# jgiovatto/srsLTE

Measured on AMD Instinct MI355X. Metric: turbo decoded Mbit/s (LTE 20 MHz, K=6144, 8 half-iterations) incl. OFDM demod of the same subframes, higher is better.
Workload: dtype int16

## Files before the change

srslte_amd/csrc/turbo_kernels.hip:

```cpp
#include <type_traits>

#include "hip_common.h"
#include "turbo_arith.h"
#include "turbo_device.h"

namespace phyhip {
namespace turbo {

typedef uint32_t u4v __attribute__((ext_vector_type(4)));
template <bool NT>
__device__ __forceinline__ uint4 ws_load16(const void* p)
{
  if constexpr (NT) {
    const u4v v = __builtin_nontemporal_load(reinterpret_cast<const u4v*>(p));
    return make_uint4(v.x, v.y, v.z, v.w);
  } else {
    return *reinterpret_cast<const uint4*>(p);
  }
}

template <class AR>
__device__ __forceinline__ void beta_step(s2 (&o)[8], s2 x, s2 y)
{
  auto adds = [](s2 a, s2 b) { return AR::add_raw(a, b); };
// ... 371 lines not shown
            y0[j] = (uint32_t)(uint16_t)AR::conv_in(r[0][3 * j + 1]) | ((uint32_t)(uint16_t)AR::conv_in(r[1][3 * j + 1]) << 16);
            y1[j] = (uint32_t)(uint16_t)AR::conv_in(r[0][3 * j + 2]) | ((uint32_t)(uint16_t)AR::conv_in(r[1][3 * j + 2]) << 16);
          }
          const uint32_t slot = (b0 + lb) * 64 + cw * LPC + pp;
          store_block_v<AR::kIs8>(S, slot, sv);
          store_block_v<AR::kIs8>(P0, slot, y0);
          store_block_v<AR::kIs8>(P1, slot, y1);
        }
      }
    }
  }
  if (pp == 0) {
    const short* in = in_wave + (size_t)(g < n_cb_left ? g : n_cb_left - 1) * in_stride;
    short*       TL = TL_wave + 16 * g;
#pragma unroll
    for (int i = 0; i < 3; i++) {
      TL[i]     = AR::conv_in(in[3 * K + 2 * i]);
      TL[3 + i] = AR::conv_in(in[3 * K + 2 * i + 1]);
      TL[6 + i] = AR::conv_in(in[3 * K + 6 + 2 * i]);
      TL[9 + i] = AR::conv_in(in[3 * K + 6 + 2 * i + 1]);
    }
  }
}

template <int LPC, class AR>
__device__ __forceinline__ void extract_input_sb16(const short* in, uint32_t K, uint32_t nblk, int lane, int pl, uint32_t* S,
                                                   uint32_t* P0, uint32_t* P1, short* TL, uint32_t* stage)
{
  constexpr int  NB  = 2 * LPC;
  const int      cbw = lane / LPC;
  uint4*         st4 = reinterpret_cast<uint4*>(stage);
  auto put = [&](uint32_t* dst, uint32_t b, const uint4& lo, const uint4& hi) {
    st4[cbw * 2 * LPC + pl]       = lo;
    st4[cbw * 2 * LPC + LPC + pl] = hi;
    uint32_t r[8];
#pragma unroll
    for (int j = 0; j < 8; j++) {
      const uint32_t w = stage[cbw * 8 * LPC + j * LPC + pl];
      r[j] = (uint32_t)(uint16_t)AR::conv_in((short)(w & 0xffffu)) | ((uint32_t)(uint16_t)AR::conv_in((short)(w >> 16)) << 16);
    }
    store_block_v<AR::kIs8>(dst, b * 64 + lane, r);
  };
  for (uint32_t b = 0; b < nblk; b++) {
    const uint4* q0 = reinterpret_cast<const uint4*>(in + (size_t)b * 8 * NB);
    const uint4* q1 = reinterpret_cast<const uint4*>(in + (size_t)(K + 32) + (size_t)b * 8 * NB);
    const uint4* q2 = reinterpret_cast<const uint4*>(in + (size_t)2 * (K + 32) + (size_t)b * 8 * NB);
    const uint4  s_lo = q0[pl], s_hi = q0[LPC + pl];
    const uint4  y_lo = q1[pl], y_hi = q1[LPC + pl];
    const uint4  z_lo = q2[pl], z_hi = q2[LPC + pl];
    put(S, b, s_lo, s_hi);
    put(P0, b, y_lo, y_hi);
    put(P1, b, z_lo, z_hi);
  }
  if (pl == 0) {
    const uint32_t tb = 3 * (K + 32);
#pragma unroll
    for (int i = 0; i < 3; i++) {
      TL[i]     = AR::conv_in(in[tb + 2 * i]);
      TL[3 + i] = AR::conv_in(in[tb + 2 * i + 1]);
      TL[6 + i] = AR::conv_in(in[tb + 6 + 2 * i]);
      TL[9 + i] = AR::conv_in(in[tb + 6 + 2 * i + 1]);
    }
  }
}

template <int LPC, class AR, bool ES, int CKS>
__device__ __forceinline__ void tdec_win_unit(const WinParams& p, const uint32_t wb, const uint32_t slab, const int lane, uint4 (&Bl)[8][2][64],
                                              uint32_t (&Tr)[512])
{
  const uint32_t crc_poly = ES ? p.crc_poly : 0u;
  const CbDesc*  desc     = ES ? p.desc : nullptr;
  constexpr int  NB  = 2 * LPC;
  constexpr int  CPW = 64 / LPC;
  constexpr bool NT  = !ES && !AR::kIs8;
  static_assert(CKS == 8 || CKS == 16, "check-points every 8 or every 16 steps");
  const int     pl   = lane % LPC;
  const int     cb_raw = (int)wb * CPW + lane / LPC;
  const bool    live = cb_raw < p.n_cb;
  const int     cb   = live ? cb_raw : p.n_cb - 1;
  const uint32_t K       = p.K;
  const uint32_t long_sb = K / NB;
  const uint32_t nblk    = (long_sb + 7) >> 3;
  const uint32_t AW      = nblk * LPC * 8;

  const uint32_t AWG = AW * CPW;
  uint32_t* ws  = p.ws + (size_t)slab * p.ws_stride * CPW;
  uint32_t* S   = ws;
  uint32_t* P0  = ws + AWG;
  uint32_t* P1  = ws + 2 * AWG;
  uint32_t* A1  = ws + 3 * AWG;
  uint32_t* D   = ws + 4 * AWG;
  uint32_t* A2  = ws + 5 * AWG;
  uint32_t* CK  = ws + 6 * AWG;
  short*    TL  = reinterpret_cast<short*>(CK + (size_t)(nblk + 1) * 64 * 8) + 16 * (lane / LPC);

  if (p.n_begin == 0) {
    const bool fast = !desc && !p.in_is8 && !p.sb_layout && (long_sb & 3u) == 0 && ((reinterpret_cast<uintptr_t>(p.input) | (2u * p.in_stride)) & 7u) == 0;
    if (fast) {
      const int first = (int)wb * CPW;
      extract_input_natural16<LPC, AR>(p.input + (size_t)first * p.in_stride, p.in_stride, p.n_cb - first, K, long_sb, nblk, lane,
                                       S, P0, P1, TL - 16 * (lane / LPC), reinterpret_cast<uint2*>(&Bl[0][0][0]));
    } else if (!p.in_is8 && p.sb_layout &&
               __all(((reinterpret_cast<uintptr_t>(p.input) + 2 * (desc ? (size_t)desc[cb].in_off : (size_t)cb * p.in_stride)) & 15u) == 0)) {
      const short* in = p.input + (desc ? (size_t)desc[cb].in_off : (size_t)cb * p.in_stride);
      extract_input_sb16<LPC, AR>(in, K, long_sb >> 3, lane, pl, S, P0, P1, TL, Tr);
      if (long_sb & 7u) {
        extract_input<LPC, AR>(in, 1, K, long_sb, nblk, lane, pl, S, P0, P1, TL, long_sb >> 3, false);
      }
    } else if (p.in_is8) {
      const signed char* in = reinterpret_cast<const signed char*>(p.input) + (desc ? (size_t)desc[cb].in_off : (size_t)cb * p.in_stride);
      extract_input<LPC, AR>(in, p.sb_layout, K, long_sb, nblk, lane, pl, S, P0, P1, TL);
    } else {
      const short* in = p.input + (desc ? (size_t)desc[cb].in_off : (size_t)cb * p.in_stride);
      extract_input<LPC, AR>(in, p.sb_layout, K, long_sb, nblk, lane, pl, S, P0, P1, TL);
    }
  }
  const uint32_t wrap_row = (AR::kIs8 && (K & 31u)) ? long_sb - 1 : 0xffffffffu;
  __syncthreads();

  uint8_t*       out       = p.output + (desc ? (size_t)desc[cb].out_off : (size_t)cb * p.out_stride);
  const uint32_t out_bytes = desc ? desc[cb].out_bytes : K / 8;
  uint32_t m_own_v = ~0u, m_row_v = ~0u;
  auto     set_masks = [&](bool dead) {
    const unsigned long long dm = __ballot(dead);
    const int                og = AR::kIs8 ? ((8 * (lane & 7)) / LPC) * LPC : ((4 * (lane & 15)) / LPC) * LPC;
    m_own_v                     = dead ? 0u : ~0u;
    m_row_v                     = ((dm >> og) & 1ull) ? 0u : ~0u;
  };
  if (ES) {
    set_masks(!live);
  }
#define M_OWN (ES ? m_own_v : ~0u)
#define M_ROW (ES ? m_row_v : ~0u)
  const bool bit_rows = !ES && p.final_run && !p.dec_llr && p.n_end > p.n_begin;
  auto decide = [&](bool write, bool final_try) -> uint32_t {
    short*         o16   = (p.dec_llr && live && write) ? p.dec_llr + (size_t)cb * K : nullptr;
    const bool     whole = (long_sb & 7) == 0;
    const uint32_t bps   = long_sb >> 3;
    const uint32_t poly  = crc_poly & 0xffffffu;
    uint32_t       c0 = 0, c1 = 0;
    const uint32_t sbs  = nblk + 1;
    uint8_t*       sbuf = reinterpret_cast<uint8_t*>(&Bl[0][0][0]) + (size_t)(lane / LPC) * NB * sbs;
    static_assert(sizeof(Bl) >= 64 / LPC * 2 * LPC * (6144 / (2 * LPC) / 8 + 2), "byte image does not fit");
    if (!whole) {
      sbuf[(2 * pl) * sbs + nblk]     = 0;
      sbuf[(2 * pl + 1) * sbs + nblk] = 0;
    }
    uint4* img = &Bl[0][0][0] + (whole ? 0u : (CPW * NB * sbs + 15u) / 16u);
    if (bit_rows) {
      for (uint32_t k = lane; k < long_sb; k += 64) {
        img[k] = ws_load16<NT>(D + (size_t)k * 4);
      }
      __syncthreads();
    }
    {
      const bool wide = whole && ((bps & 3) == 0) && ((reinterpret_cast<uintptr_t>(out) & 3) == 0) && out_bytes == K / 8;
      uint32_t   w0 = 0, w1 = 0;
      uint32_t   t[8], tn[8];
      if (!bit_rows) {
        issue_rows_raw<AR::kIs8, NT>(D, 0, lane, t);
      }
      for (uint32_t b = 0; b < nblk; b++) {
        if (!bit_rows && b + 1 < nblk) {
          issue_rows_raw<AR::kIs8, NT>(D, (b + 1) & M_ROW, lane, tn);
        }
        uint32_t r[8];
        if (bit_rows) {
#pragma unroll
          for (int j = 0; j < 8; j++) {
            const uint32_t k = b * 8 + j < long_sb ? b * 8 + j : long_sb - 1;
            const uint4    m = img[k];
            r[j] = (uint32_t)(((((uint64_t)m.y << 32) | m.x) >> lane) & 1u) | ((uint32_t)(((((uint64_t)m.w << 32) | m.z) >> lane) & 1u) << 16);
          }
        } else {
          rows_to_lane_v<AR::kIs8>(Tr, lane, t, r);
        }
        uint32_t b0 = 0, b1 = 0;
#pragma unroll
        for (int j = 0; j < 8; j++) {
          if (b * 8 + j < long_sb) {
            const s2       v  = from_u(r[j]);
            const uint32_t x0 = v.x > 0 ? 1u : 0u, x1 = v.y > 0 ? 1u : 0u;
            b0 |= (x0 << 7) >> j;
            b1 |= (x1 << 7) >> j;
            if (crc_poly) {
              c0 = ((c0 << 1) & 0xffffffu) ^ ((((c0 >> 23) ^ x0) & 1u) ? poly : 0u);
              c1 = ((c1 << 1) & 0xffffffu) ^ ((((c1 >> 23) ^ x1) & 1u) ? poly : 0u);
            }
            if (o16 && whole) {
              o16[(2 * pl) * long_sb + b * 8 + j]     = AR::out16(v.x);
              o16[(2 * pl + 1) * long_sb + b * 8 + j] = AR::out16(v.y);
            }
          }
        }
        if (!whole) {
          sbuf[(2 * pl) * sbs + b]     = (uint8_t)b0;
          sbuf[(2 * pl + 1) * sbs + b] = (uint8_t)b1;
        }
        if (whole && write && live) {
          if (wide) {
            w0 |= b0 << (8 * (b & 3));
            w1 |= b1 << (8 * (b & 3));
            if ((b & 3) == 3) {
              *reinterpret_cast<uint32_t*>(out + (2 * pl) * bps + (b & ~3u))     = w0;
              *reinterpret_cast<uint32_t*>(out + (2 * pl + 1) * bps + (b & ~3u)) = w1;
              w0 = w1 = 0;
            }
          } else {
            if ((2 * pl) * bps + b < out_bytes) {
              out[(2 * pl) * bps + b] = (uint8_t)b0;
            }
            if ((2 * pl + 1) * bps + b < out_bytes) {
              out[(2 * pl + 1) * bps + b] = (uint8_t)b1;
            }
          }
        }
        if (!bit_rows) {
#pragma unroll
          for (int j = 0; j < 8; j++) {
            t[j] = tn[j];
          }
        }
      }
    }
    uint32_t crc = 0;
    if (crc_poly) {
      auto mulmod = [&](uint32_t a, uint32_t m) {
        uint32_t r = 0;
#pragma unroll 4
        for (int i = 23; i >= 0; i--) {
          r = ((r << 1) & 0xffffffu) ^ (((r >> 23) & 1u) ? poly : 0u);
          r ^= ((m >> i) & 1u) ? a : 0u;
        }
        return r;
      };
      crc = mulmod(c0, p.crc_mult[2 * pl]) ^ mulmod(c1, p.crc_mult[2 * pl + 1]);
#pragma unroll
      for (int off = LPC / 2; off > 0; off >>= 1) {
        crc ^= __shfl_xor(crc, off, LPC);
      }
    }
    __syncthreads();
    if (!whole && write && (!crc_poly || crc == 0 || final_try)) {
      const uint32_t nbytes = K / 8;
      const uint32_t lim    = out_bytes < nbytes ? out_bytes : nbytes;
      const bool     al     = (reinterpret_cast<uintptr_t>(out) & 3) == 0;
      for (uint32_t w = pl; w * 4 < nbytes; w += LPC) {
        uint32_t d = (w * 32) / long_sb, k = w * 32 - d * long_sb;
        uint32_t word = 0;
#pragma unroll
        for (int t = 0; t < 4; t++) {
          if (w * 4 + t < nbytes) {
            const uint8_t* q = sbuf + d * sbs + (k >> 3);
            uint32_t       v = ((((uint32_t)q[0] << 8) | q[1]) >> (8 - (k & 7))) & 0xffu;
            if (k + 8 > long_sb && d + 1 < (uint32_t)NB) {
              v |= (uint32_t)sbuf[(d + 1) * sbs] >> (long_sb - k);
            }
            word |= v << (8 * t);
          }
          k += 8;
          if (k >= long_sb) {
            k -= long_sb;
            d++;
          }
        }
        if (live) {
          if (al && w * 4 + 3 < lim) {
            *reinterpret_cast<uint32_t*>(out + 4 * w) = word;
          } else {
#pragma unroll
            for (int t = 0; t < 4; t++) {
              if (w * 4 + t < lim) {
                out[w * 4 + t] = (uint8_t)(word >> (8 * t));
              }
            }
          }
        }
      }
      if (o16) {
        const short* sd = reinterpret_cast<const short*>(D);
        for (uint32_t nn = pl; nn < K; nn += LPC) {
          const uint32_t d = nn / long_sb, k = nn % long_sb;
          const uint32_t e = (k * 64 + (lane / LPC) * LPC + (d >> 1)) * 2 + (d & 1);
          o16[nn] = AR::kIs8 ? (short)reinterpret_cast<const signed char*>(D)[e] : sd[e];
        }
      }
    }
    __syncthreads();
    return crc;
  };
  bool     done = false;
  uint32_t noi  = 0;

  for (uint32_t n = p.n_begin; n < p.n_end; n++) {
    const bool      dec1    = !(n & 1);
    const bool      has_app = dec1 && n > 0;
    const uint32_t* Y       = dec1 ? P0 : P1;
    const short*    xt      = dec1 ? TL : TL + 6;
    const short*    yt      = dec1 ? TL + 3 : TL + 9;

    struct Ops {
      uint32_t x[8], y[8], a[8];
    };
    auto issue = [&](uint32_t b, Ops& q) {
      if (dec1) {
        load_block_raw<AR::kIs8, NT>(S, (b & M_OWN) * 64 + lane, q.x);
      } else {
        issue_rows_raw<AR::kIs8, NT>(A2, b & M_ROW, lane, q.x);
      }
      load_block_raw<AR::kIs8, NT>(Y, (b & M_OWN) * 64 + lane, q.y);
      if (has_app) {
        issue_rows_raw<AR::kIs8, NT>(A1, b & M_ROW, lane, q.a);
      }
    };
    auto prep = [&](const Ops& q, s2(&xs)[8], s2(&ys)[8], s2(&ap)[8]) {
      uint32_t xr[8], ar[8], yr[8];
      if (dec1) {
        block_values<AR::kIs8>(q.x, xr);
      } else {
        rows_to_lane_v<AR::kIs8>(Tr, lane, q.x, xr);
      }
      if (has_app) {
        rows_to_lane_v<AR::kIs8>(Tr, lane, q.a, ar);
      }
      block_values<AR::kIs8>(q.y, yr);
#pragma unroll
      for (int j = 0; j < 8; j++) {
        xs[j] = from_u(xr[j]);
        ys[j] = from_u(yr[j]);
        ap[j] = splat(0);
        if (has_app) {
          ap[j] = from_u(ar[j]);
          xs[j] = AR::add(ap[j], xs[j]);
        }
      }
    };
    auto taken = [&](const Ops& q) {
      asm volatile("" ::"v"(q.x[0]), "v"(q.x[1]), "v"(q.x[2]), "v"(q.x[3]), "v"(q.x[4]), "v"(q.x[5]), "v"(q.x[6]), "v"(q.x[7]));
      asm volatile("" ::"v"(q.y[0]), "v"(q.y[1]), "v"(q.y[2]), "v"(q.y[3]), "v"(q.y[4]), "v"(q.y[5]), "v"(q.y[6]), "v"(q.y[7]));
      if (has_app) {
        asm volatile("" ::"v"(q.a[0]), "v"(q.a[1]), "v"(q.a[2]), "v"(q.a[3]), "v"(q.a[4]), "v"(q.a[5]), "v"(q.a[6]), "v"(q.a[7]));
      }
    };
    Ops cur, nxt, nx2;

    s2 fw[8];
#pragma unroll
    for (int i = 0; i < 8; i++) {
      fw[i] = splat(-AR::kInf);
    }
    {
      const uint32_t w0 = long_sb - TD_WIN_OVERLAP;
      const uint32_t bl = nblk - 1;
      issue(w0 >> 3, cur);
      for (uint32_t b = w0 >> 3; b <= bl; b++) {
        issue(b < bl ? b + 1 : TD_WIN_OVERLAP / 8 - 1, nxt);
        s2 xs[8], ys[8], ap[8];
        prep(cur, xs, ys, ap);
        if (b + 4 > bl) {
          const uint32_t s = b + 3 - bl;
          Bl[2 * s][0][lane]     = make_uint4(to_u(xs[0]), to_u(xs[1]), to_u(xs[2]), to_u(xs[3]));
          Bl[2 * s][1][lane]     = make_uint4(to_u(xs[4]), to_u(xs[5]), to_u(xs[6]), to_u(xs[7]));
          Bl[2 * s + 1][0][lane] = make_uint4(to_u(ys[0]), to_u(ys[1]), to_u(ys[2]), to_u(ys[3]));
          Bl[2 * s + 1][1][lane] = make_uint4(to_u(ys[4]), to_u(ys[5]), to_u(ys[6]), to_u(ys[7]));
        }
#pragma unroll
        for (int j = 0; j < 8; j++) {
          uint32_t k = b * 8 + j;
          if (k >= w0 && k < long_sb) {
            alpha_step<AR, false>(fw, fw, xs[j], ys[j]);
            uint32_t kk = k - w0;
            if (AR::norm_at(kk)) {
              AR::normalize(fw);
            }
          }
        }
        cur = nxt;
      }
    }
#pragma unroll
    for (int i = 0; i < 8; i++) {
      uint32_t u   = to_u(fw[i]);
      uint32_t prv = __shfl_up(u, 1, LPC);
      uint32_t lo  = (pl == 0) ? (uint32_t)(uint16_t)(short)(i ? -AR::kInf : 0) : (prv >> 16);
      uint32_t hi  = u & 0xffffu;
      fw[i]        = from_u(lo | (hi << 16));
    }

    s2 o[8];
#pragma unroll
    for (int i = 0; i < 8; i++) {
      o[i] = splat(-AR::kInf);
    }
    for (int b = TD_WIN_OVERLAP / 8 - 1; b >= 0; b--) {
      if (b > 0) {
        issue(b - 1, nxt);
      }
      s2 xs[8], ys[8], ap[8];
      prep(cur, xs, ys, ap);
#pragma unroll
      for (int j = 7; j >= 0; j--) {
        beta_step<AR>(o, xs[j], ys[j]);
        uint32_t k = b * 8 + j;
        if (AR::norm_at(k)) {
          AR::normalize(o);
        }
      }
      cur = nxt;
    }
    {
      short tr[8];
      tail_trellis<AR>(xt, yt, tr);
#pragma unroll
      for (int i = 0; i < 8; i++) {
        uint32_t u   = to_u(o[i]);
        uint32_t nxt = __shfl_down(u, 1, LPC);
        uint32_t lo  = u >> 16;
        uint32_t hi  = (pl == LPC - 1) ? (uint32_t)(uint16_t)tr[i] : (nxt & 0xffffu);
        o[i]         = from_u(lo | (hi << 16));
      }
      uint32_t ck[8];
#pragma unroll
      for (int i = 0; i < 8; i++) {
        ck[i] = to_u(o[i]);
      }
      store_block_v<AR::kIs8>(CK, (nblk & M_OWN) * 64 + lane, ck);
    }
    for (int b = (int)nblk - 1; b >= 0; b--) {
      const bool ahead = b + 3 <= (int)nblk;
      if (b > 1 && ahead) {
        issue(b - 2, nx2);
      }
      s2 xs[8], ys[8], ap[8];
      if (b + 4 >= (int)nblk) {
        const uint32_t s  = (uint32_t)b + 4 - nblk;
        const uint4    x0 = Bl[2 * s][0][lane], x1 = Bl[2 * s][1][lane], y0 = Bl[2 * s + 1][0][lane], y1 = Bl[2 * s + 1][1][lane];
        xs[0] = from_u(x0.x), xs[1] = from_u(x0.y), xs[2] = from_u(x0.z), xs[3] = from_u(x0.w);
        xs[4] = from_u(x1.x), xs[5] = from_u(x1.y), xs[6] = from_u(x1.z), xs[7] = from_u(x1.w);
        ys[0] = from_u(y0.x), ys[1] = from_u(y0.y), ys[2] = from_u(y0.z), ys[3] = from_u(y0.w);
        ys[4] = from_u(y1.x), ys[5] = from_u(y1.y), ys[6] = from_u(y1.z), ys[7] = from_u(y1.w);
      } else {
        prep(cur, xs, ys, ap);
      }
#pragma unroll
      for (int j = 7; j >= 0; j--) {
        uint32_t k = b * 8 + j;
        if (k < long_sb) {
          beta_step<AR>(o, xs[j], ys[j]);
          if (j == 0 && b > 0 && (CKS == 8 || !(b & 1))) {
            uint32_t ck[8];
#pragma unroll
            for (int i = 0; i < 8; i++) {
              ck[i] = to_u(o[i]);
            }
            store_block_v<AR::kIs8>(CK, ((uint32_t)b & M_OWN) * 64 + lane, ck);
          }
          if (AR::norm_at(k)) {
            AR::normalize(o);
          }
        }
      }
      if (b > 0 && ahead) {
        cur = nxt;
        nxt = nx2;
      }
    }
    __syncthreads();

#pragma unroll
    for (int i = 0; i < 8; i++) {
      o[i] = fw[i];
    }

    const uint32_t* lut = dec1 ? p.deint : p.inter;
    uint32_t*       dst = dec1 ? A2 : A1;
    const bool fuse = dec1 && n >= 2;
    const bool last = (n + 1 == p.n_end) || crc_poly;
    const bool fin  = bit_rows && n + 1 == p.n_end;

    auto rederive = [&](uint32_t b, int len, const s2(&xs)[8], const s2(&ys)[8], const uint32_t(&ckv)[8]) {
      s2 st[8];
#pragma unroll
      for (int i = 0; i < 8; i++) {
        st[i] = from_u(ckv[i]);
      }
      Bl[len - 1][0][lane] = make_uint4(ckv[0], ckv[1], ckv[2], ckv[3]);
      Bl[len - 1][1][lane] = make_uint4(ckv[4], ckv[5], ckv[6], ckv[7]);
#pragma unroll
      for (int j = 6; j >= 0; j--) {
        if (j <= len - 2) {
          uint32_t idx = b * 8 + j + 2;
          if (idx != long_sb && AR::norm_at(idx)) {
            AR::normalize(st);
          }
          beta_step<AR>(st, xs[j + 1], ys[j + 1]);
          Bl[j][0][lane] = make_uint4(to_u(st[0]), to_u(st[1]), to_u(st[2]), to_u(st[3]));
          Bl[j][1][lane] = make_uint4(to_u(st[4]), to_u(st[5]), to_u(st[6]), to_u(st[7]));
        }
      }
    };
    auto emit = [&](uint32_t b, int len, const s2(&xs)[8], const s2(&ys)[8], const s2(&ap)[8], const uint32_t(&tr)[8]) {
      uint32_t outv[8], rawv[8];
#pragma unroll
      for (int j = 0; j < 8; j++) {
        outv[j] = 0;
        rawv[j] = 0;
        if (j < len) {
          const uint4 b0 = Bl[j][0][lane], b1 = Bl[j][1][lane];
          const s2    B[8] = {from_u(b0.x), from_u(b0.y), from_u(b0.z), from_u(b0.w),
                              from_u(b1.x), from_u(b1.y), from_u(b1.z), from_u(b1.w)};
          s2       llr = alpha_step<AR, true>(o, B, xs[j], ys[j]);
          uint32_t k   = b * 8 + j;
          if (AR::norm_at(k)) {
            AR::normalize(o);
          }
          s2 proc = llr;
          if (fuse) {
            proc = AR::ex_sub(llr, ap[j], k == wrap_row);
          } else if (!dec1) {
            proc = AR::ex_sub(llr, xs[j], (tr[j] & 0xffffu) == wrap_row);
          }
          outv[j] = to_u(proc);
          rawv[j] = to_u(llr);
        }
      }
      if constexpr (CKS == 16) {
        asm volatile("" ::"v"(tr[0]), "v"(tr[1]), "v"(tr[2]), "v"(tr[3]), "v"(tr[4]), "v"(tr[5]), "v"(tr[6]), "v"(tr[7]));
      }
#pragma unroll
      for (int j = 0; j < 8; j++) {
        if (j < len) {
          const uint32_t row = tr[j] & 0xffffu & M_OWN;
          if (fin) {
            const s2       v  = from_u(dec1 ? rawv[j] : permute_pair<LPC>(rawv[j], tr[j] >> 16));
            const uint64_t mx = __ballot(v.x > 0), my = __ballot(v.y > 0);
            if (lane == 0) {
              *reinterpret_cast<uint4*>(D + (size_t)(dec1 ? b * 8 + j : row) * 4) =
                  make_uint4((uint32_t)mx, (uint32_t)(mx >> 32), (uint32_t)my, (uint32_t)(my >> 32));
            }
            continue;
          }
          store_row<AR::kIs8>(dst, row, lane, permute_pair<LPC>(outv[j], tr[j] >> 16));
          if (last) {
            if (dec1) {
              store_row<AR::kIs8>(D, (b * 8 + j) & M_OWN, lane, rawv[j]);
            } else {
              store_row<AR::kIs8>(D, row, lane, permute_pair<LPC>(rawv[j], tr[j] >> 16));
            }
          }
        }
      }
    };

    if constexpr (CKS == 8) {
      uint32_t ck[8], tr[8], ckn[8], trn[8];
      load_block_raw<AR::kIs8, NT>(CK, (1u & M_OWN) * 64 + lane, ck);
      load_lut(lut, pl, tr);
      if (nblk > 1) {
        issue(1, nxt);
      }
      for (uint32_t b = 0; b < nblk; b++) {
        const int len = (long_sb - b * 8) < 8 ? (int)(long_sb - b * 8) : 8;
        s2        xs[8], ys[8], ap[8];
        if (b + 2 < nblk) {
          issue(b + 2, nx2);
        }
        if (b + 1 < nblk) {
          load_block_raw<AR::kIs8, NT>(CK, ((b + 2) & M_OWN) * 64 + lane, ckn);
          load_lut(lut, (b + 1) * LPC + pl, trn);
        }
        prep(cur, xs, ys, ap);
        uint32_t ckv[8];
        block_values<AR::kIs8>(ck, ckv);
        rederive(b, len, xs, ys, ckv);
        emit(b, len, xs, ys, ap, tr);
        cur = nxt;
        nxt = nx2;
#pragma unroll
        for (int i = 0; i < 8; i++) {
          ck[i] = ckn[i];
          tr[i] = trn[i];
        }
      }
    } else {
      Ops&     q0 = cur;
      Ops&     q1 = nxt;
      Ops&     q2 = nx2;
      Ops      q3;
      uint32_t ck[8], tr[8];
      load_block_raw<AR::kIs8, NT>(CK, ((nblk < 2 ? nblk : 2u) & M_OWN) * 64 + lane, ck);
      if (nblk > 1) {
        issue(1, q1);
      }
      if (nblk > 2) {
        issue(2, q2);
      }
      auto block = [&](auto even, uint32_t b, const Ops& c, const Ops& held, Ops& tgt) {
        const int len = (long_sb - b * 8) < 8 ? (int)(long_sb - b * 8) : 8;
        s2       xs[8], ys[8], ap[8];
        uint32_t  ckv[8];
        asm volatile("" ::"v"(ck[0]), "v"(ck[1]), "v"(ck[2]), "v"(ck[3]), "v"(ck[4]), "v"(ck[5]), "v"(ck[6]), "v"(ck[7]));
        block_values<AR::kIs8>(ck, ckv);
        taken(c);
        if constexpr (even.value) {
          const bool paired = b + 1 < nblk;
          s2        x1[8], y1[8], a1[8];
          if (paired) {
            taken(held);
            prep(held, x1, y1, a1);
          }
          prep(c, xs, ys, ap);
          if (b + 3 < nblk) {
            issue(b + 3, tgt);
          }
          load_lut(lut, b * LPC + pl, tr);
          if (paired) {
            const int len1 = (long_sb - (b + 1) * 8) < 8 ? (int)(long_sb - (b + 1) * 8) : 8;
            s2       st[8];
#pragma unroll
            for (int i = 0; i < 8; i++) {
              st[i] = from_u(ckv[i]);
            }
#pragma unroll
            for (int j = 7; j >= 0; j--) {
              if (j < len1) {
                uint32_t idx = (b + 1) * 8 + j + 1;
                if (idx != long_sb && AR::norm_at(idx)) {
                  AR::normalize(st);
                }
                beta_step<AR>(st, x1[j], y1[j]);
              }
            }
#pragma unroll
            for (int i = 0; i < 8; i++) {
              ckv[i] = to_u(st[i]);
            }
          }
          rederive(b, len, xs, ys, ckv);
        } else {
          prep(c, xs, ys, ap);
          if (b + 3 < nblk) {
            issue(b + 3, tgt);
          }
          load_lut(lut, b * LPC + pl, tr);
          rederive(b, len, xs, ys, ckv);
          const uint32_t bn = b + 3 < nblk ? b + 3 : nblk;
          load_block_raw<AR::kIs8, NT>(CK, (bn & M_OWN) * 64 + lane, ck);
        }
        emit(b, len, xs, ys, ap, tr);
      };
      constexpr std::integral_constant<bool, true>  kEven{};
      constexpr std::integral_constant<bool, false> kOdd{};
      for (uint32_t b = 0; b < nblk; b += 4) {
        block(kEven, b, q0, q1, q3);
        if (b + 1 < nblk) {
          block(kOdd, b + 1, q1, q2, q0);
        }
        if (b + 2 < nblk) {
          block(kEven, b + 2, q2, q3, q1);
        }
        if (b + 3 < nblk) {
          block(kOdd, b + 3, q3, q0, q2);
        }
      }
    }
    __syncthreads();
    if (crc_poly) {
      const bool     fin = n + 1 == p.n_end;
      const bool     wr  = !done;
      const uint32_t crc = decide(wr, fin);
      if (!done) {
        noi++;
        done = crc == 0;
      }
      set_masks(done || !live);
      __syncthreads();
      if (__all(done || !live) || fin) {
        break;
      }
    }
  }

#undef M_OWN
#undef M_ROW
  if (!crc_poly) {
    decide(true, true);
  } else if (p.noi && live && pl == 0) {
    p.noi[cb_raw]    = (int)noi;
    p.crc_ok[cb_raw] = done ? 1 : 0;
  }
}

template <class AR, bool ES>
constexpr int win_ck_spacing = (!AR::kIs8 && !ES) ? 16 : 8;

template <int LPC, class AR, bool ES, int CKS = win_ck_spacing<AR, ES>>
__global__ __launch_bounds__(64) __attribute__((amdgpu_waves_per_eu(2, 2))) void tdec_win_kernel(const WinParams p)
{
  __shared__ uint4    Bl[8][2][64];
  __shared__ uint32_t Tr[512];
  tdec_win_unit<LPC, AR, ES, CKS>(p, blockIdx.x, blockIdx.x, threadIdx.x, Bl, Tr);
}

#ifdef SRSRAN_HIP_WITH_VARIANTS
__global__ __launch_bounds__(64) __attribute__((amdgpu_waves_per_eu(1, 1))) void tdec_win_kernel_waves1(const WinParams p)
{
  __shared__ uint4    Bl[8][2][64];
  __shared__ uint32_t Tr[512];
  tdec_win_unit<8, Ar16, false, win_ck_spacing<Ar16, false>>(p, blockIdx.x, blockIdx.x, threadIdx.x, Bl, Tr);
}
__global__ __launch_bounds__(64) __attribute__((amdgpu_waves_per_eu(2, 2))) void tdec_win_kernel_persistent(const WinParams p)
{
  __shared__ uint4    Bl[8][2][64];
  __shared__ uint32_t Tr[512];
  uint32_t wb = blockIdx.x;
  while (wb < p.n_units) {
    auto ka = __builtin_amdgcn_kernarg_segment_ptr();
    asm volatile("" : "+s"(ka));
    const WinParams& q = *(const WinParams*)ka;
    int lane = threadIdx.x;
    asm volatile("" : "+v"(lane));
    tdec_win_unit<8, Ar16, false, win_ck_spacing<Ar16, false>>(q, wb, blockIdx.x, lane, Bl, Tr);
    __syncthreads();
    uint32_t nx = 0;
    if (threadIdx.x == 0) {
      nx = gridDim.x + atomicAdd(q.unit_counter, 1u);
    }
    wb = (uint32_t)__builtin_amdgcn_readfirstlane((int)nx);
  }
}

#endif
__device__ __forceinline__ void gen_acs_beta(short (&old)[8], short x, short y)
{
  short xy = wrap16(x + y);
  short m_b[8], nw[8];
  m_b[0] = wrap16(old[4] + xy);
  m_b[1] = old[4];
  m_b[2] = wrap16(old[5] + y);
  m_b[3] = wrap16(old[5] + x);
  m_b[4] = wrap16(old[6] + x);
  m_b[5] = wrap16(old[6] + y);
  m_b[6] = old[7];
  m_b[7] = wrap16(old[7] + xy);
  nw[0] = old[0];
  nw[1] = wrap16(old[0] + xy);
  nw[2] = wrap16(old[1] + x);
  nw[3] = wrap16(old[1] + y);
  nw[4] = wrap16(old[2] + y);
  nw[5] = wrap16(old[2] + x);
  nw[6] = wrap16(old[3] + xy);
  nw[7] = old[3];
#pragma unroll
  for (int i = 0; i < 8; i++) {
    old[i] = m_b[i] > nw[i] ? m_b[i] : nw[i];
  }
}

__global__ __launch_bounds__(64) void tdec_gen_kernel(const GenParams p)
{
  const int lane = threadIdx.x;
  const int cb   = blockIdx.x * 64 + lane;
  if (cb >= p.n_cb) {
    return;
  }
  const uint32_t K  = p.K;
  const uint32_t L  = K + 4;
  short* ws = p.ws + (size_t)blockIdx.x * p.ws_stride;
#define GV(base, idx) ws[((size_t)(base) + (idx)) * 64 + lane]
  const uint32_t oS = 0, oP0 = L, oP1 = 2 * L, oA1 = 3 * L, oA2 = 4 * L, oE1 = 5 * L, oE2 = 6 * L, oB = 7 * L;

  if (p.n_begin == 0) {
    const size_t       in_off = p.desc ? (size_t)p.desc[cb].in_off : (size_t)cb * p.in_stride;
    const short*       in16 = p.input + in_off;
    const signed char* in8  = reinterpret_cast<const signed char*>(p.input) + in_off;
    auto               in   = [&](uint32_t i) -> short { return p.in_is8 ? (short)in8[i] : in16[i]; };
    for (uint32_t i = 0; i < K; i++) {
      GV(oS, i)  = in(3 * i);
      GV(oP0, i) = in(3 * i + 1);
      GV(oP1, i) = in(3 * i + 2);
    }
    for (uint32_t i = K; i < K + 3; i++) {
      GV(oS, i)  = in(3 * K + 2 * (i - K));
      GV(oP0, i) = in(3 * K + 2 * (i - K) + 1);
      GV(oA2, i) = in(3 * K + 6 + 2 * (i - K));
      GV(oP1, i) = in(3 * K + 6 + 2 * (i - K) + 1);
    }
  }
  const uint16_t* inter   = p.inter;
  const uint16_t* deinter = p.deinter;
  uint32_t        n_run    = p.n_end;
  bool            crc_good = false;

  for (uint32_t n = p.n_begin; n < p.n_end; n++) {
    const bool     dec1    = !(n & 1);
    const bool     has_app = dec1 && n > 0;
    const uint32_t oX = dec1 ? oS : oA2, oY = dec1 ? oP0 : oP1, oOut = dec1 ? oE1 : oE2;
    if (dec1) {
      if (n) {
        for (uint32_t i = 0; i < K; i++) {
          GV(oA1, i) = wrap16(GV(oA1, i) - GV(oE1, i));
        }
      }
    } else {
      for (uint32_t i = 0; i < K; i++) {
        short e = GV(oE1, i);
        if (n > 1) {
          e          = wrap16(e - GV(oA1, i));
          GV(oE1, i) = e;
        }
        GV(oA2, deinter[i]) = e;
      }
    }
    short old[8];
    old[0] = 0;
#pragma unroll
    for (int i = 1; i < 8; i++) {
      old[i] = -TD_INF;
    }
    const uint32_t end = K + 3;
#pragma unroll
    for (int i = 0; i < 8; i++) {
      GV(oB + 8 * end, i) = old[i];
    }
    for (int k = (int)end - 1; k >= 0; k--) {
      short x = GV(oX, k);
      if (has_app && (uint32_t)k < K) {
        x = wrap16(x + GV(oA1, k));
      }
      short y = GV(oY, k);
      gen_acs_beta(old, x, y);
#pragma unroll
      for (int i = 0; i < 8; i++) {
        GV(oB + 8 * k, i) = old[i];
      }
      if ((k % 4) == 0 && (uint32_t)k < K) {
#pragma unroll
        for (int i = 1; i < 8; i++) {
          old[i] = wrap16(old[i] - old[0]);
        }
        old[0] = 0;
      }
    }
    old[0] = 0;
#pragma unroll
    for (int i = 1; i < 8; i++) {
      old[i] = -TD_INF;
    }
    for (uint32_t k = 1; k < K + 1; k++) {
      short x = GV(oX, k - 1);
      if (has_app) {
        x = wrap16(x + GV(oA1, k - 1));
      }
      short y  = GV(oY, k - 1);
      short xy = wrap16(x + y);
      short m_b[8], nw[8];
      m_b[0] = old[0];
      m_b[1] = wrap16(old[3] + y);
      m_b[2] = wrap16(old[4] + y);
      m_b[3] = old[7];
      m_b[4] = old[1];
      m_b[5] = wrap16(old[2] + y);
      m_b[6] = wrap16(old[5] + y);
      m_b[7] = old[6];
      nw[0] = wrap16(old[1] + xy);
      nw[1] = wrap16(old[2] + x);
      nw[2] = wrap16(old[5] + x);
      nw[3] = wrap16(old[6] + xy);
      nw[4] = wrap16(old[0] + xy);
      nw[5] = wrap16(old[3] + x);
      nw[6] = wrap16(old[4] + x);
      nw[7] = wrap16(old[7] + xy);
      short m1 = 0, m0 = 0;
#pragma unroll
      for (int i = 0; i < 8; i++) {
        short bq = GV(oB + 8 * k, i);
        short v0 = wrap16(m_b[i] + bq);
        short v1 = wrap16(nw[i] + bq);
        m0 = (i == 0) ? v0 : (v0 > m0 ? v0 : m0);
        m1 = (i == 0) ? v1 : (v1 > m1 ? v1 : m1);
      }
#pragma unroll
      for (int i = 0; i < 8; i++) {
        old[i] = m_b[i] > nw[i] ? m_b[i] : nw[i];
      }
      if ((k % 4) == 0) {
#pragma unroll
        for (int i = 1; i < 8; i++) {
          old[i] = wrap16(old[i] - old[0]);
        }
        old[0] = 0;
      }
      GV(oOut, k - 1) = wrap16(m1 - m0);
    }
    if (!dec1) {
      for (uint32_t i = 0; i < K; i++) {
        GV(oA1, inter[i]) = GV(oE2, i);
      }
    }
    n_run = n + 1;
    if (p.crc_poly) {
      const uint32_t oC = (n_run & 1) ? oE1 : oA1;
      const uint32_t g  = p.crc_poly & 0xffffffu;
      uint32_t       c  = 0;
      for (uint32_t i = 0; i < K; i++) {
        const uint32_t x = GV(oC, i) > 0 ? 1u : 0u;
        c = ((c << 1) & 0xffffffu) ^ ((((c >> 23) ^ x) & 1u) ? g : 0u);
      }
      if (c == 0) {
        crc_good = true;
        break;
      }
    }
  }
  if (p.noi) {
    p.noi[cb] = (int)(n_run - p.n_begin);
  }
  if (p.crc_ok) {
    p.crc_ok[cb] = crc_good ? 1 : 0;
  }
  const uint32_t oD        = (n_run & 1) ? oE1 : oA1;
  uint8_t*       out       = p.output + (p.desc ? (size_t)p.desc[cb].out_off : (size_t)cb * p.out_stride);
  const uint32_t out_bytes = p.desc ? p.desc[cb].out_bytes : K / 8;
  for (uint32_t jb = 0; jb < out_bytes; jb++) {
    uint32_t byte = 0;
#pragma unroll
    for (int t = 0; t < 8; t++) {
      byte |= (GV(oD, jb * 8 + t) > 0 ? 0x80u : 0u) >> t;
    }
    out[jb] = (uint8_t)byte;
  }
  if (p.dec_llr) {
    short* o16 = p.dec_llr + (size_t)cb * K;
    for (uint32_t i = 0; i < K; i++) {
      o16[i] = GV(oD, i);
    }
  }
#undef GV
}



template <bool ES>
static hipError_t launch_win_es(int nb, bool arith8, const WinParams& p, hipStream_t stream)
{
  const int lpc = nb / 2;
  dim3      grid(ceil_div(p.n_cb, 64 / lpc));
#ifdef SRSRAN_HIP_WITH_VARIANTS
  if (!ES && !arith8 && nb == 16 && p.variant == 1) {
    hipLaunchKernelGGL(tdec_win_kernel_waves1, grid, dim3(64), 0, stream, p);
  } else if (!ES && !arith8 && nb == 16 && p.variant == 2 && p.unit_counter) {
    hipLaunchKernelGGL(tdec_win_kernel_persistent, dim3(p.n_units < p.max_resident ? p.n_units : p.max_resident), dim3(64), 0, stream, p);
  } else
#endif
  if (!arith8 && nb == 16) {
    hipLaunchKernelGGL((tdec_win_kernel<8, Ar16, ES>), grid, dim3(64), 0, stream, p);
  } else if (!arith8 && nb == 8) {
    hipLaunchKernelGGL((tdec_win_kernel<4, Ar16, ES>), grid, dim3(64), 0, stream, p);
  } else if (arith8 && nb == 16) {
    hipLaunchKernelGGL((tdec_win_kernel<8, Ar8, ES>), grid, dim3(64), 0, stream, p);
  } else if (arith8 && nb == 32) {
    hipLaunchKernelGGL((tdec_win_kernel<16, Ar8, ES>), grid, dim3(64), 0, stream, p);
  } else {
    return hipErrorInvalidValue;
  }
  return hipGetLastError();
// ... 22 lines not shown
```

Baseline: 36140.

## Unroll beta recursion by four with rotating load buffers and predicated prefetch

For the 16-step checkpoint variant, the backward beta pass becomes a 4-way unrolled loop with four rotating operand buffers, so block operands are prefetched three blocks ahead without register copies. Out-of-range prefetches are predicated into dummy loads instead of branches. The alpha/emit loop is reordered to issue loads and LUT reads earlier, and the tail guards are removed so the loop body stays uniform. This is meant to hide global-load latency better in the serial trellis recursion, at the cost of more registers and some redundant loads past the end of the block.

New measurement: 37360, median of 6. 3.4% higher.

```diff
diff --git a/srslte_amd/csrc/turbo_kernels.hip b/srslte_amd/csrc/turbo_kernels.hip
--- a/srslte_amd/csrc/turbo_kernels.hip
+++ b/srslte_amd/csrc/turbo_kernels.hip
@@ -697,15 +697,27 @@
     struct Ops {
       uint32_t x[8], y[8], a[8];
     };
-    auto issue = [&](uint32_t b, Ops& q) {
-      if (dec1) {
-        load_block_raw<AR::kIs8, NT>(S, (b & M_OWN) * 64 + lane, q.x);
+    const uint32_t* X = dec1 ? S : A2;
+    auto issue = [&](uint32_t b, Ops& q, bool ok = true) {
+      if constexpr (CKS == 16) {
+        static_assert(!ES, "the early-stop masks differ between blocked and row arrays");
+        const bool oka = ok && has_app;
+        uint32_t   bb = ok ? b : 0u, ba = oka ? b : 0u;
+        int        ln = ok ? lane : 0, la = oka ? lane : 0;
+        asm volatile("" : "+v"(ln), "+v"(la));
+        issue_rows_raw<AR::kIs8, NT>(X, bb, ln, q.x);
+        issue_rows_raw<AR::kIs8, NT>(Y, bb, ln, q.y);
+        issue_rows_raw<AR::kIs8, NT>(A1, ba, la, q.a);
       } else {
-        issue_rows_raw<AR::kIs8, NT>(A2, b & M_ROW, lane, q.x);
-      }
-      load_block_raw<AR::kIs8, NT>(Y, (b & M_OWN) * 64 + lane, q.y);
-      if (has_app) {
-        issue_rows_raw<AR::kIs8, NT>(A1, b & M_ROW, lane, q.a);
+        if (dec1) {
+          load_block_raw<AR::kIs8, NT>(S, (b & M_OWN) * 64 + lane, q.x);
+        } else {
+          issue_rows_raw<AR::kIs8, NT>(A2, b & M_ROW, lane, q.x);
+        }
+        load_block_raw<AR::kIs8, NT>(Y, (b & M_OWN) * 64 + lane, q.y);
+        if (has_app) {
+          issue_rows_raw<AR::kIs8, NT>(A1, b & M_ROW, lane, q.a);
+        }
       }
     };
     auto prep = [&](const Ops& q, s2(&xs)[8], s2(&ys)[8], s2(&ap)[8]) {
@@ -733,11 +745,11 @@
     auto taken = [&](const Ops& q) {
       asm volatile("" ::"v"(q.x[0]), "v"(q.x[1]), "v"(q.x[2]), "v"(q.x[3]), "v"(q.x[4]), "v"(q.x[5]), "v"(q.x[6]), "v"(q.x[7]));
       asm volatile("" ::"v"(q.y[0]), "v"(q.y[1]), "v"(q.y[2]), "v"(q.y[3]), "v"(q.y[4]), "v"(q.y[5]), "v"(q.y[6]), "v"(q.y[7]));
-      if (has_app) {
+      if (has_app || CKS == 16) {
         asm volatile("" ::"v"(q.a[0]), "v"(q.a[1]), "v"(q.a[2]), "v"(q.a[3]), "v"(q.a[4]), "v"(q.a[5]), "v"(q.a[6]), "v"(q.a[7]));
       }
     };
-    Ops cur, nxt, nx2;
+    Ops cur, nxt, nx2, nx3;
 
     s2 fw[8];
 #pragma unroll
@@ -821,43 +833,88 @@
       }
       store_block_v<AR::kIs8>(CK, (nblk & M_OWN) * 64 + lane, ck);
     }
-    for (int b = (int)nblk - 1; b >= 0; b--) {
-      const bool ahead = b + 3 <= (int)nblk;
-      if (b > 1 && ahead) {
-        issue(b - 2, nx2);
-      }
-      s2 xs[8], ys[8], ap[8];
-      if (b + 4 >= (int)nblk) {
-        const uint32_t s  = (uint32_t)b + 4 - nblk;
-        const uint4    x0 = Bl[2 * s][0][lane], x1 = Bl[2 * s][1][lane], y0 = Bl[2 * s + 1][0][lane], y1 = Bl[2 * s + 1][1][lane];
-        xs[0] = from_u(x0.x), xs[1] = from_u(x0.y), xs[2] = from_u(x0.z), xs[3] = from_u(x0.w);
-        xs[4] = from_u(x1.x), xs[5] = from_u(x1.y), xs[6] = from_u(x1.z), xs[7] = from_u(x1.w);
-        ys[0] = from_u(y0.x), ys[1] = from_u(y0.y), ys[2] = from_u(y0.z), ys[3] = from_u(y0.w);
-        ys[4] = from_u(y1.x), ys[5] = from_u(y1.y), ys[6] = from_u(y1.z), ys[7] = from_u(y1.w);
-      } else {
-        prep(cur, xs, ys, ap);
-      }
-#pragma unroll
-      for (int j = 7; j >= 0; j--) {
-        uint32_t k = b * 8 + j;
-        if (k < long_sb) {
-          beta_step<AR>(o, xs[j], ys[j]);
-          if (j == 0 && b > 0 && (CKS == 8 || !(b & 1))) {
-            uint32_t ck[8];
-#pragma unroll
-            for (int i = 0; i < 8; i++) {
-              ck[i] = to_u(o[i]);
-            }
-            store_block_v<AR::kIs8>(CK, ((uint32_t)b & M_OWN) * 64 + lane, ck);
-          }
-          if (AR::norm_at(k)) {
-            AR::normalize(o);
-          }
-        }
-      }
-      if (b > 0 && ahead) {
-        cur = nxt;
-        nxt = nx2;
+    if constexpr (CKS == 16) {
+      const int top = (int)nblk - 5;
+      auto      block = [&](int b, const Ops& c, Ops& tgt) {
+        s2 xs[8], ys[8], ap[8];
+        if (b > top) {
+          const uint32_t s  = (uint32_t)(b < (int)nblk ? b : (int)nblk - 1) + 4 - nblk;
+          const uint4    x0 = Bl[2 * s][0][lane], x1 = Bl[2 * s][1][lane], y0 = Bl[2 * s + 1][0][lane], y1 = Bl[2 * s + 1][1][lane];
+          xs[0] = from_u(x0.x), xs[1] = from_u(x0.y), xs[2] = from_u(x0.z), xs[3] = from_u(x0.w);
+          xs[4] = from_u(x1.x), xs[5] = from_u(x1.y), xs[6] = from_u(x1.z), xs[7] = from_u(x1.w);
+          ys[0] = from_u(y0.x), ys[1] = from_u(y0.y), ys[2] = from_u(y0.z), ys[3] = from_u(y0.w);
+          ys[4] = from_u(y1.x), ys[5] = from_u(y1.y), ys[6] = from_u(y1.z), ys[7] = from_u(y1.w);
+        } else {
+          taken(c);
+          prep(c, xs, ys, ap);
+        }
+        issue(b - 3, tgt, b >= 3 && b - 3 <= top);
+        if (b < (int)nblk) {
+#pragma unroll
+          for (int j = 7; j >= 0; j--) {
+            uint32_t k = b * 8 + j;
+            if (k < long_sb) {
+              beta_step<AR>(o, xs[j], ys[j]);
+              if (j == 0 && b > 0 && !(b & 1)) {
+                uint32_t ck[8];
+#pragma unroll
+                for (int i = 0; i < 8; i++) {
+                  ck[i] = to_u(o[i]);
+                }
+                store_block_v<AR::kIs8>(CK, ((uint32_t)b & M_OWN) * 64 + lane, ck);
+              }
+              if (AR::norm_at(k)) {
+                AR::normalize(o);
+              }
+            }
+          }
+        }
+      };
+      for (int b = ((int)nblk - 1) | 3; b >= 0; b -= 4) {
+        block(b, nx3, cur);
+        block(b - 1, nx2, nx3);
+        block(b - 2, nxt, nx2);
+        block(b - 3, cur, nxt);
+      }
+    } else {
+      for (int b = (int)nblk - 1; b >= 0; b--) {
+        const bool ahead = b + 3 <= (int)nblk;
+        if (b > 1 && ahead) {
+          issue(b - 2, nx2);
+        }
+        s2 xs[8], ys[8], ap[8];
+        if (b + 4 >= (int)nblk) {
+          const uint32_t s  = (uint32_t)b + 4 - nblk;
+          const uint4    x0 = Bl[2 * s][0][lane], x1 = Bl[2 * s][1][lane], y0 = Bl[2 * s + 1][0][lane], y1 = Bl[2 * s + 1][1][lane];
+          xs[0] = from_u(x0.x), xs[1] = from_u(x0.y), xs[2] = from_u(x0.z), xs[3] = from_u(x0.w);
+          xs[4] = from_u(x1.x), xs[5] = from_u(x1.y), xs[6] = from_u(x1.z), xs[7] = from_u(x1.w);
+          ys[0] = from_u(y0.x), ys[1] = from_u(y0.y), ys[2] = from_u(y0.z), ys[3] = from_u(y0.w);
+          ys[4] = from_u(y1.x), ys[5] = from_u(y1.y), ys[6] = from_u(y1.z), ys[7] = from_u(y1.w);
+        } else {
+          prep(cur, xs, ys, ap);
+        }
+#pragma unroll
+        for (int j = 7; j >= 0; j--) {
+          uint32_t k = b * 8 + j;
+          if (k < long_sb) {
+            beta_step<AR>(o, xs[j], ys[j]);
+            if (j == 0 && b > 0 && (CKS == 8 || !(b & 1))) {
+              uint32_t ck[8];
+#pragma unroll
+              for (int i = 0; i < 8; i++) {
+                ck[i] = to_u(o[i]);
+              }
+              store_block_v<AR::kIs8>(CK, ((uint32_t)b & M_OWN) * 64 + lane, ck);
+            }
+            if (AR::norm_at(k)) {
+              AR::normalize(o);
+            }
+          }
+        }
+        if (b > 0 && ahead) {
+          cur = nxt;
+          nxt = nx2;
+        }
       }
     }
     __syncthreads();
@@ -873,14 +930,16 @@
     const bool last = (n + 1 == p.n_end) || crc_poly;
     const bool fin  = bit_rows && n + 1 == p.n_end;
 
-    auto rederive = [&](uint32_t b, int len, const s2(&xs)[8], const s2(&ys)[8], const uint32_t(&ckv)[8]) {
-      s2 st[8];
+    auto rederive_start = [&](int len, const uint32_t(&ckv)[8], s2(&st)[8]) {
 #pragma unroll
       for (int i = 0; i < 8; i++) {
         st[i] = from_u(ckv[i]);
       }
-      Bl[len - 1][0][lane] = make_uint4(ckv[0], ckv[1], ckv[2], ckv[3]);
-      Bl[len - 1][1][lane] = make_uint4(ckv[4], ckv[5], ckv[6], ckv[7]);
+      const int top = CKS == 16 ? (len - 1) & 7 : len - 1;
+      Bl[top][0][lane] = make_uint4(ckv[0], ckv[1], ckv[2], ckv[3]);
+      Bl[top][1][lane] = make_uint4(ckv[4], ckv[5], ckv[6], ckv[7]);
+    };
+    auto rederive_rest = [&](uint32_t b, int len, const s2(&xs)[8], const s2(&ys)[8], s2(&st)[8]) {
 #pragma unroll
       for (int j = 6; j >= 0; j--) {
         if (j <= len - 2) {
@@ -894,7 +953,7 @@
         }
       }
     };
-    auto emit = [&](uint32_t b, int len, const s2(&xs)[8], const s2(&ys)[8], const s2(&ap)[8], const uint32_t(&tr)[8]) {
+    auto emit = [&](uint32_t b, int len, const s2(&xs)[8], const s2(&ys)[8], const s2(&ap)[8], const uint32_t(&tr)[8], auto&& ck_taken) {
       uint32_t outv[8], rawv[8];
 #pragma unroll
       for (int j = 0; j < 8; j++) {
@@ -921,6 +980,7 @@
       }
       if constexpr (CKS == 16) {
         asm volatile("" ::"v"(tr[0]), "v"(tr[1]), "v"(tr[2]), "v"(tr[3]), "v"(tr[4]), "v"(tr[5]), "v"(tr[6]), "v"(tr[7]));
+        ck_taken();
       }
 #pragma unroll
       for (int j = 0; j < 8; j++) {
@@ -967,8 +1027,10 @@
         prep(cur, xs, ys, ap);
         uint32_t ckv[8];
         block_values<AR::kIs8>(ck, ckv);
-        rederive(b, len, xs, ys, ckv);
-        emit(b, len, xs, ys, ap, tr);
+        s2 st[8];
+        rederive_start(len, ckv, st);
+        rederive_rest(b, len, xs, ys, st);
+        emit(b, len, xs, ys, ap, tr, [] {});
         cur = nxt;
         nxt = nx2;
 #pragma unroll
@@ -981,82 +1043,75 @@
       Ops&     q0 = cur;
       Ops&     q1 = nxt;
       Ops&     q2 = nx2;
-      Ops      q3;
+      Ops&     q3 = nx3;
       uint32_t ck[8], tr[8];
       load_block_raw<AR::kIs8, NT>(CK, ((nblk < 2 ? nblk : 2u) & M_OWN) * 64 + lane, ck);
-      if (nblk > 1) {
-        issue(1, q1);
-      }
-      if (nblk > 2) {
-        issue(2, q2);
-      }
+      issue(1, q1, nblk > 1);
+      asm volatile("" ::"v"(ck[0]), "v"(ck[1]), "v"(ck[2]), "v"(ck[3]), "v"(ck[4]), "v"(ck[5]), "v"(ck[6]), "v"(ck[7]));
+      taken(q1);
+      issue(2, q2, nblk > 2);
       auto block = [&](auto even, uint32_t b, const Ops& c, const Ops& held, Ops& tgt) {
-        const int len = (long_sb - b * 8) < 8 ? (int)(long_sb - b * 8) : 8;
-        s2       xs[8], ys[8], ap[8];
-        uint32_t  ckv[8];
-        asm volatile("" ::"v"(ck[0]), "v"(ck[1]), "v"(ck[2]), "v"(ck[3]), "v"(ck[4]), "v"(ck[5]), "v"(ck[6]), "v"(ck[7]));
+        const int rem = (int)long_sb - (int)b * 8;
+        const int len = rem < 0 ? 0 : rem < 8 ? rem : 8;
+        s2         xs[8], ys[8], ap[8], st[8];
+        uint32_t   ckv[8];
+        auto       ck_taken = [&] { asm volatile("" ::"v"(ck[0]), "v"(ck[1]), "v"(ck[2]), "v"(ck[3]), "v"(ck[4]), "v"(ck[5]), "v"(ck[6]), "v"(ck[7])); };
+        ck_taken();
         block_values<AR::kIs8>(ck, ckv);
+        load_lut(lut, (b < nblk ? b : nblk - 1) * LPC + pl, tr);
         taken(c);
         if constexpr (even.value) {
-          const bool paired = b + 1 < nblk;
-          s2        x1[8], y1[8], a1[8];
-          if (paired) {
-            taken(held);
-            prep(held, x1, y1, a1);
-          }
-          prep(c, xs, ys, ap);
-          if (b + 3 < nblk) {
-            issue(b + 3, tgt);
-          }
-          load_lut(lut, b * LPC + pl, tr);
-          if (paired) {
-            const int len1 = (long_sb - (b + 1) * 8) < 8 ? (int)(long_sb - (b + 1) * 8) : 8;
-            s2       st[8];
-#pragma unroll
-            for (int i = 0; i < 8; i++) {
-              st[i] = from_u(ckv[i]);
-            }
-#pragma unroll
-            for (int j = 7; j >= 0; j--) {
-              if (j < len1) {
-                uint32_t idx = (b + 1) * 8 + j + 1;
-                if (idx != long_sb && AR::norm_at(idx)) {
-                  AR::normalize(st);
-                }
-                beta_step<AR>(st, x1[j], y1[j]);
-              }
-            }
-#pragma unroll
-            for (int i = 0; i < 8; i++) {
-              ckv[i] = to_u(st[i]);
-            }
-          }
-          rederive(b, len, xs, ys, ckv);
+          taken(held);
+          issue(b + 3, tgt, b + 3 < nblk);
         } else {
           prep(c, xs, ys, ap);
-          if (b + 3 < nblk) {
-            issue(b + 3, tgt);
-          }
-          load_lut(lut, b * LPC + pl, tr);
-          rederive(b, len, xs, ys, ckv);
+          rederive_start(len, ckv, st);
           const uint32_t bn = b + 3 < nblk ? b + 3 : nblk;
           load_block_raw<AR::kIs8, NT>(CK, (bn & M_OWN) * 64 + lane, ck);
-        }
-        emit(b, len, xs, ys, ap, tr);
+          issue(b + 3, tgt, b + 3 < nblk);
+        }
+        {
+          if constexpr (even.value) {
+            const bool paired = b + 1 < nblk;
+            s2        x1[8], y1[8], a1[8];
+            if (paired) {
+              prep(held, x1, y1, a1);
+            }
+            prep(c, xs, ys, ap);
+            if (paired) {
+              const int len1 = (long_sb - (b + 1) * 8) < 8 ? (int)(long_sb - (b + 1) * 8) : 8;
+#pragma unroll
+              for (int i = 0; i < 8; i++) {
+                st[i] = from_u(ckv[i]);
+              }
+#pragma unroll
+              for (int j = 7; j >= 0; j--) {
+                if (j < len1) {
+                  uint32_t idx = (b + 1) * 8 + j + 1;
+                  if (idx != long_sb && AR::norm_at(idx)) {
+                    AR::normalize(st);
+                  }
+                  beta_step<AR>(st, x1[j], y1[j]);
+                }
+              }
+#pragma unroll
+              for (int i = 0; i < 8; i++) {
+                ckv[i] = to_u(st[i]);
+              }
+            }
+            rederive_start(len, ckv, st);
+          }
+          rederive_rest(b, len, xs, ys, st);
+          emit(b, len, xs, ys, ap, tr, ck_taken);
+        }
       };
       constexpr std::integral_constant<bool, true>  kEven{};
       constexpr std::integral_constant<bool, false> kOdd{};
       for (uint32_t b = 0; b < nblk; b += 4) {
         block(kEven, b, q0, q1, q3);
-        if (b + 1 < nblk) {
-          block(kOdd, b + 1, q1, q2, q0);
-        }
-        if (b + 2 < nblk) {
-          block(kEven, b + 2, q2, q3, q1);
-        }
-        if (b + 3 < nblk) {
-          block(kOdd, b + 3, q3, q0, q2);
-        }
+        block(kOdd, b + 1, q1, q2, q0);
+        block(kEven, b + 2, q2, q3, q1);
+        block(kOdd, b + 3, q3, q0, q2);
       }
     }
     __syncthreads();
```
